# godhj93/bayesian-torch

Measured on AMD Instinct MI355X. Metric: MC-samples/sec (forward+KL), Bayesian-ResNet18 CIFAR batch=128, higher is better.
Workload: dtype f32 (bf16x3 split operands, 6 product terms, f32 accumulate); 1 GPU; cfg3: Bayesian-ResNet18 via dnn_to_bnn (Conv2dReparameterization), CIFAR 3x32x32, batch=128; samples_per_launch=32, batch=128, rng=on-chip philox, parallelism=mc1, output_stage=bn+relu+residual (+ the stem max-pool) folded into the conv kernels, launch=hip graph replay

## Files before the change

### bayesian_torch_amd/_lib.py

```python
import ctypes as C
import os
import threading

import torch

_HERE = os.path.dirname(os.path.abspath(__file__))
LIB_PATH = os.environ.get("BT_LIB_PATH") or os.path.join(_HERE, "libbtorch_hip.so")
WORKSPACE_BYTES = 65536
KL_MAX_SEGMENTS = 64
PACK_MAX_SEGMENTS = 64
KL_RHO_IS_SIGMA = 1
KL_PRIOR_LAPLACE = 2
PRIOR_NORMAL, PRIOR_LAPLACE = 0, 1
DRAWS_EPS_PACKED = 1
LOWRANK_MAX_R = 4
DRAWS_SIGNS_PACKED = 2


def signs_packed_stride(n):
    return (int(n) + 15) // 16 * 16

_f32p = C.POINTER(C.c_float)
_vp = C.c_void_p

# ... 56 lines not shown
class bt_minmax_seg(C.Structure):
    _fields_ = [("x", _vp), ("n", C.c_int64), ("dst", _vp)]


MINMAX_MAX_SEGS = 4

_lib = None
_lock = threading.Lock()

_FWD_TAIL = [_vp, C.c_int64, C.POINTER(bt_params), C.POINTER(bt_draws), C.POINTER(bt_epilogue), _vp, _vp, _vp, C.c_size_t, _vp]
_PROTOS = {
    "bt_version": (C.c_int, []),
    "bt_last_error_string": (C.c_char_p, []),
    "bt_last_kernel_name": (C.c_char_p, []),
    "bt_last_launch_info": (C.c_int, [C.POINTER(C.c_int64), C.c_int32]),
    "bt_fused_scratch_bytes": (C.c_size_t, [C.POINTER(bt_conv2d_geom), C.c_int32]),
    "bt_set_contraction": (C.c_int, [C.c_int]),
    "bt_get_contraction": (C.c_int, []),
    "bt_conv2d_bwd_workspace": (C.c_size_t, [C.POINTER(bt_conv2d_geom), C.c_int32]),
    "bt_conv2d_bwd": (C.c_int, [C.POINTER(bt_conv2d_geom), C.c_int32, C.c_int32, _vp, C.c_int64, _vp, C.POINTER(bt_params), C.POINTER(bt_draws),
                                _vp, _vp, _vp, _vp, C.c_size_t, _vp]),
    "bt_maxpool_3x3s2": (C.c_int, [_vp, _vp, C.c_int64, C.c_int32, C.c_int32, _vp]),
    "bt_conv2d_bwd_kl": (C.c_int, [C.POINTER(bt_conv2d_geom), C.c_int32, C.c_int32, _vp, C.c_int64, _vp, C.POINTER(bt_params), C.POINTER(bt_draws), _vp,
                                   _vp, _vp, _vp, _vp, C.c_size_t, _vp]),
    "bt_kl_normal_bwd": (C.c_int, [_vp, _vp, _vp, _vp, _vp, C.c_int64, C.c_uint32, _vp, _vp, _vp]),
    "bt_kl_normal_bwd_segs": (C.c_int, [C.c_int32, C.POINTER(_vp), C.POINTER(_vp), C.POINTER(_vp), C.POINTER(_vp), C.POINTER(C.c_int64), _vp, C.c_uint32,
                                        C.POINTER(_vp), C.POINTER(_vp), _vp]),
    "bt_reparam_linear_fwd": (C.c_int, [C.c_int32] * 4 + _FWD_TAIL),
    "bt_flipout_linear_fwd": (C.c_int, [C.c_int32] * 4 + _FWD_TAIL),
    "bt_reparam_conv2d_fwd": (C.c_int, [C.POINTER(bt_conv2d_geom), C.c_int32] + _FWD_TAIL),
# ... 72 lines not shown
                    fn = getattr(handle, name)
                    fn.restype, fn.argtypes = res, args
                _lib = handle
    return _lib


LAUNCH_INFO_FIELDS = ("workgroups", "m_tiles", "n_tiles", "S", "t_NI", "t_R", "t_Wt", "pixel_major", "row_tiles", "kl_slices", "groups", "n_bt", "n_rt", "n_ct", "fused_kl")


def last_launch_info():
    v = (C.c_int64 * 16)()
    check(lib().bt_last_launch_info(v, 16))
    return dict(zip(LAUNCH_INFO_FIELDS, (int(x) for x in v)))


ERR_UNSUPPORTED = -2


def check(rc):
    if rc != 0:
        raise RuntimeError(f"libbtorch_hip error {rc}: {lib().bt_last_error_string().decode()}")


def ptr(t):
    return None if t is None else t.data_ptr()


def dev_f32(t, what):
    if t is None:
        return None
# ... 96 lines not shown
```

### bayesian_torch_amd/csrc/bt_fused_api.hip

```cpp
#include <math.h>
#include <string.h>

#include "bt_fused_fwd.h"

namespace bt {
typedef int Launcher(bool linear, const FwdArgs& a, FwdArgs& ran, hipStream_t stream);
Launcher launch_reparam, launch_reparam_inj, launch_reparam_updil, launch_reparam_dwin, launch_flipout, launch_flipout_inj, launch_flipout_updil, launch_flipout_dwin;
static Launcher* const kLaunchers[2][4] = {{launch_reparam, launch_reparam_inj, launch_reparam_updil, launch_reparam_dwin},
                                           {launch_flipout, launch_flipout_inj, launch_flipout_updil, launch_flipout_dwin}};

EnvKnob g_force_generic{"BT_FORCE_GENERIC", [](const char* e) { return e ? 1 : 0; }};
static unsigned long long* g_dbg = nullptr;
static thread_local long long g_launch_info[16] = {};
static inline bool al16(const void* p) { return (((uintptr_t)p) & 15u) == 0; }
static void record_plan(const FwdArgs& r, int fused_kl) {
  const long long v[16] = {r.total_blocks, r.m_tiles, r.n_tiles, r.S, r.t_NI, r.t_R, r.t_Wt, r.pixel_major, r.row_taps, r.kl_slices, r.G, r.n_bt, r.n_rt, r.n_ct, fused_kl, 0};
  for (int i = 0; i < 16; ++i) g_launch_info[i] = v[i];
}

struct Call {
  bool flip, linear;
  const bt_conv2d_geom& g;
  int S;
  const float* x;
  int64_t x_sample_stride;
  const bt_params* p;
  const bt_draws* d;
  const bt_epilogue* ep;
  float *out, *kl_out;
  void* ws;
  size_t ws_bytes;
  const char* who;
  const bt_updil* u;
// ... 343 lines not shown
```

### bayesian_torch_amd/csrc/bt_fused_common.h

```cpp
#pragma once
#include "bt_api_internal.h"

namespace bt {

struct FwdArgs {
  const float *x, *mu_w, *rho_w, *mu_b, *rho_b, *pmu_w, *psig_w, *pmu_b, *psig_b;
  const float *mu_pk, *sig_pk;
  const float *eps_w, *eps_b, *sign_in, *sign_out;
  float* out;
  float* kl_out;
  double* slots;
  unsigned* counter;
  long long x_sample_stride, x_elems, out_elems, w_elems;
  int B, Ci, H, W, Co, KH, KW, SH, SW, PH, PW, DH, DW, G;
  int Ho, Wo, HoWo, M, K, Cig, Cog, S, T, HW;
  int n_tiles, m_tiles, total_blocks;
  int t_NI, t_R, t_Wt, n_bt, n_rt, n_ct;
  int patch_ok;
  int x_cvec;
  int x_rows;
  int pixel_major, mt_per_pixel;
  int w_vec, x_vec;
  int do_kl, kl_slices;
  uint32_t seed_lo, seed_hi, call, layer_id, sample0;
  const uint32_t* call_base;
  const float *ep_scale, *ep_shift, *ep_res;
  long long ep_res_stride;
  int ep_relu;
  int ep_pool, ep_Hp, ep_Wp;
  int out_vec4;
  int bn32;
  unsigned long long* dbg;
  uint32_t inv_m_tiles, inv_S, inv_n_tiles, inv_n_bt, inv_n_ct, inv_rw, inv_wt, inv_kw;
  int x_flat;
  int row_taps;
  float* sk_scratch;
  unsigned* sk_tickets;
  long long sk_scratch_bytes;
  int sk_nsl, sk_ks, sk_cpt;
// ... 21 lines not shown
  constexpr size_t end_dw = offsetof(FwdArgs, inv_do) + sizeof(uint32_t);
  constexpr size_t end_lr = offsetof(FwdArgs, lr_R) + sizeof(int);
  constexpr size_t end_obs = offsetof(FwdArgs, obs_nonfinite) + sizeof(unsigned*);
  static_assert(offsetof(FwdArgs, call_base) == hole + 4 && offsetof(FwdArgs, dwin) == end && offsetof(FwdArgs, lowrank) == end_dw &&
                    offsetof(FwdArgs, obs_dst) == end_lr && sizeof(FwdArgs) == end_obs,
                "FwdArgs padding moved: name the holes here");
  h = fnv1a(h, &a, hole);
  h = fnv1a(h, &a.call_base, end - offsetof(FwdArgs, call_base));
  if (a.dwin) h = fnv1a(h, &a.dwin, end_dw - end);
  if (a.lowrank) h = fnv1a(h, &a.lowrank, end_lr - end_dw);
  return a.obs_nonfinite ? fnv1a(h, &a.obs_dst, end_obs - end_lr) : h;
}

int launch_split(FwdArgs a, FwdArgs& ran, hipStream_t stream);
int launch_split_flip(FwdArgs a, FwdArgs& ran, hipStream_t stream);
int contraction_mode();
long long skinny_scratch_bytes(const bt_conv2d_geom& g, int S);

__device__ __forceinline__ RngKey weight_key(const FwdArgs& a) {
  RngKey key_w;
  key_w.seed_lo = a.seed_lo;
  key_w.seed_hi = a.seed_hi;
  key_w.call = a.call + (a.call_base ? __builtin_nontemporal_load(a.call_base) : 0u);
  key_w.layer_tensor = layer_tensor_word(a.layer_id, 0);
  return key_w;
}

__device__ __forceinline__ void sign_keys(const FwdArgs& a, const RngKey& key_w, uint32_t sample, uint32_t* skey_in, uint32_t* skey_out) {
  RngKey ks = key_w;
  ks.layer_tensor = layer_tensor_word(a.layer_id, 2);
// ... 103 lines not shown
  bt_ = wave_sum(bt_);
  if (lane == 0) {
    float kl = (float)(t / (double)a.w_elems);
    if (a.mu_b) kl += (float)(bt_ / (double)a.Co);
    a.kl_out[0] = kl;
    __hip_atomic_store(a.counter, 0u, __ATOMIC_RELAXED, __HIP_MEMORY_SCOPE_AGENT);
  }
}
__device__ __forceinline__ double kl_slot_sum(const FwdArgs& a, int nslots, int lane) {
  double t = 0.0;
  for (int q = lane; q < nslots; q += 64) t += __hip_atomic_load(&a.slots[q], __ATOMIC_RELAXED, __HIP_MEMORY_SCOPE_AGENT);
  for (int q = lane; q < nslots; q += 64) __hip_atomic_store(&a.slots[q], 0.0, __ATOMIC_RELAXED, __HIP_MEMORY_SCOPE_AGENT);
  return t;
}

struct ColDecode {
  int b0, r0, w0, RW, Mt, t_Wt;
  uint32_t inv_rw, inv_wt;
  int B, Ho, Wo;
  __device__ __forceinline__ bool decode(int ml, int& b, int& ho, int& wo) const {
    const int img = RW == 1 ? ml : (int)__umulhi((uint32_t)ml, inv_rw);
    const int rem = ml - img * RW;
    const int r = t_Wt == 1 ? rem : (int)__umulhi((uint32_t)rem, inv_wt);
    b = b0 + img, ho = r0 + r, wo = w0 + (rem - r * t_Wt);
    return ml < Mt && b < B && ho < Ho && wo < Wo;
  }
};

}
```

### bayesian_torch_amd/csrc/bt_fused_split.h

```cpp
#pragma once
#include "bt_fused_common.h"
#include "bt_fused_fwd.h"

namespace bt {

typedef short bf16x8 __attribute__((ext_vector_type(8)));

constexpr int kSplitSteps = 5;

template <int BM, bool FLIP = false>
constexpr int split_xpo() {
  return FLIP ? 302 : 1025;
}
template <int BN, int NP, bool FLIP = false>
constexpr int split_w_bytes() { return (FLIP ? 2 : 1) * kSplitSteps * 2 * NP * BN * 16; }
template <int BM, int NP, bool FLIP = false>
constexpr int split_x_bytes() { return split_xpo<BM, FLIP>() * (NP + (FLIP ? 1 : 0)) * 16; }
constexpr int kSplitMiscBytes = kMaxTaps * 16 + 96 + 32 + 64;
template <int BN, int BM, int NP, bool FLIP = false>
constexpr int split_stage_cap() {
  constexpr int ops = 2 * (split_w_bytes<BN, NP, FLIP>() + split_x_bytes<BM, NP, FLIP>()), pass32 = (4 * BN + 32 * (BM + 4)) * 4;
  return (NP == 1 && pass32 > ops) ? pass32 : ops;
}
template <int BN, int BM, int NP, bool FLIP = false>
// ... 30 lines not shown
  return inv ? (int)__umulhi((uint32_t)n, inv) : (d == 1 ? n : n / d);
}
__device__ __forceinline__ uint32_t inv32(int d) { return 0xFFFFFFFFu / (uint32_t)d + 1u; }
__device__ __forceinline__ int div_small(int n, int d) { return d == 1 ? n : d == 2 ? n >> 1 : n / d; }

#ifndef BT_ONE_PIXEL_STEPS
#define BT_ONE_PIXEL_STEPS 4
#endif
constexpr int kOnePixelSteps = BT_ONE_PIXEL_STEPS;

__device__ __forceinline__ uint32_t guarded_off(bool in, uint32_t off) {
  const uint32_t m = 0u - (uint32_t)in;
  return (off & m) | (0x80000000u & ~m);
}

__device__ __forceinline__ bool one_pixel_tile(const FwdArgs& a, int* tap) {
  if (a.HoWo != 1 || a.HW != 1 || a.t_R != 1 || a.t_Wt != 1 || a.m_tiles != a.n_bt || a.updil) return false;
  const int kh = a.DH == 1 ? a.PH : a.PH / a.DH, kw = a.DW == 1 ? a.PW : a.PW / a.DW;
  *tap = kh * a.KW + kw;
  return kh * a.DH == a.PH && kh < a.KH && kw * a.DW == a.PW && kw < a.KW && (a.Cig >> 3) > 0;
}

template <int BN, int NP, int NPW, bool INJ>
__device__ __forceinline__ void split_one_pixel_tile(const FwdArgs& a, const int tap) {
  constexpr int BM = 128, KS = kOnePixelSteps, kProducers = 64 * NPW, TN = BN / 32;
  constexpr int W_STEP = 2 * NP * BN * 16, W_HALF = NP * BN * 16, W_PIECE = BN * 16, W_RING = KS * W_STEP;
  constexpr int XD = 4;
  static_assert(KS % XD == 0, "whole groups per stage");
  static_assert(2 * W_RING + 3 * BN * 4 <= split_stage_cap<BN, BM, NP>(), "two weight images + the channel constants fit the operand buffers");
  extern __shared__ __attribute__((aligned(16))) char smem_c[];
  float* const bias0 = reinterpret_cast<float*>(smem_c + 2 * W_RING);
// ... 302 lines not shown
  const int mt = __builtin_amdgcn_readfirstlane(L - Lq * a.m_tiles);
  L = Lq, Lq = udiv_inv(L, a.S, a.inv_S);
  const int s = __builtin_amdgcn_readfirstlane(L - Lq * a.S);
  L = Lq, Lq = udiv_inv(L, a.n_tiles, a.inv_n_tiles);
  const int nt = __builtin_amdgcn_readfirstlane(L - Lq * a.n_tiles);
  const int g = __builtin_amdgcn_readfirstlane(Lq);
  const int n0 = nt * BN;
  const bool pix = a.pixel_major != 0;
  const int t_NI = a.t_NI, t_R = a.t_R, t_Wt = a.t_Wt, RW = t_R * t_Wt, Mt = t_NI * RW;
  const int trest = udiv_inv(mt, a.n_bt, a.inv_n_bt);
  const int bt = __builtin_amdgcn_readfirstlane(mt - trest * a.n_bt);
  const int rt = __builtin_amdgcn_readfirstlane(udiv_inv(trest, a.n_ct, a.inv_n_ct)), ct = __builtin_amdgcn_readfirstlane(trest - rt * a.n_ct);
  const int b0 = bt * t_NI, r0 = rt * t_R, w0 = ct * t_Wt;
  const uint32_t inv_rw = RW > 1 ? (a.inv_rw ? a.inv_rw : inv32(RW)) : 0u;
  const uint32_t inv_wt = t_Wt > 1 ? (a.inv_wt ? a.inv_wt : inv32(t_Wt)) : 0u;
  const ColDecode cols = {b0, r0, w0, RW, Mt, t_Wt, inv_rw, inv_wt, a.B, a.Ho, a.Wo};
  const uint32_t sample = a.sample0 + (uint32_t)s;
  const int T = a.T, Cig = a.Cig;

  const RngKey key_w = weight_key(a);
  uint32_t skey_in = 0, skey_out = 0;
  if constexpr (FLIP) sign_keys(a, key_w, sample, &skey_in, &skey_out);

  int nA, dymin, dymax, dxmin, dxmax;
  {
    bool act = false;
    int4 e = make_int4(0, 0, 0, 0);
    if (lane < T) {
      const int kh = udiv_inv(lane, a.KW, a.inv_kw), kw = lane - kh * a.KW;
      e = make_int4(0, kh * a.DH, kw * a.DW, lane);
      if (pix) {
// ... 144 lines not shown
      for (int u = 0; u < U; ++u) {
        if (relu) v[u].x = v[u].x < 0.f ? 0.f : v[u].x, v[u].y = v[u].y < 0.f ? 0.f : v[u].y, v[u].z = v[u].z < 0.f ? 0.f : v[u].z, v[u].w = v[u].w < 0.f ? 0.f : v[u].w;
        if (okq[u]) *reinterpret_cast<float4*>(out_s + oidx[u]) = v[u];
      }
    }
  };

  const bool stage_cols = !a.out_vec4 && !pix && !a.row_taps && a.Ho * a.Wo > 4;
  auto readout_cols = [&](int pass, int t0) {
    constexpr int SROW = BM + 4, NT_ = kThreadsAll;
    static_assert(NT_ % BM == 0, "a thread keeps its column");
    constexpr int RSTEP = NT_ / BM, NITc = (SROWS + RSTEP - 1) / RSTEP;
    const float* const stage = smem + 4 * BN;
    const int c = t0 % BM, row0 = t0 / BM;
    int bq, hq, wq;
    const bool mok = cols.decode(c, bq, hq, wq);
    const int HoWo_ = a.Ho * a.Wo;
    const int co0 = pass * SROWS + row0;
    const uint32_t obase = mok ? (uint32_t)(((bq * a.Co + g * a.Cog + n0 + co0) * a.Ho + hq) * a.Wo + wq) : 0u;
    const int rows_ok = a.Cog - n0 - pass * SROWS < SROWS ? a.Cog - n0 - pass * SROWS : SROWS;
    const float* const sp = stage + row0 * SROW + c;
#pragma unroll 8
    for (int k = 0; k < NITc; ++k) {
      const int row = row0 + k * RSTEP;
      const bool ok = mok && row < rows_ok;
      const uint32_t oi = ok ? obase + (uint32_t)(k * RSTEP * HoWo_) : 0u;
      const int rr = row < SROWS ? k * RSTEP : 0;
      float v = sp[rr * SROW];
      if constexpr (FLIP) {
        const float d = sp[(SROWS + rr) * SROW];
        const int co_l = ok ? co0 + k * RSTEP : 0;
// ... 424 lines not shown
    auto kl_ticket = [&]() {
      int last = 0;
      if (lane == 0) last = (__hip_atomic_fetch_add(a.counter, 1u, __ATOMIC_RELAXED, __HIP_MEMORY_SCOPE_AGENT) == (unsigned)a.kl_slices - 1u) ? 1 : 0;
      if (__builtin_amdgcn_readfirstlane(last))
        kl_close(a, kl_slot_sum(a, 4 * a.kl_slices, lane), lane);
    };
    int xaddr[TM][kSplitSteps];
    {
      int pimg[TM], pyb[TM], pxb[TM];
      bool live[TM];
#pragma unroll
      for (int j = 0; j < TM; ++j) {
        int b, ho, wo;
        live[j] = cols.decode(wm * WTM + j * 32 + li, b, ho, wo);
        pimg[j] = (b - b0) * PIMG, pyb[j] = (ho - r0) * ps_h, pxb[j] = (wo - w0) * ps_w;
      }
#pragma unroll
      for (int q = 0; q < kSplitSteps; ++q) {
        int ol, ai;
        if (nA <= 1) ol = 2 * q + lh, ai = 0;
        else ol = (q >= SPO) + (q >= 2 * SPO) + (q >= 3 * SPO) + (q >= 4 * SPO), ai = 2 * (q - ol * SPO) + lh;
        const bool ent = nA > 0 && ol < NO && ai < nA;
        const int4 e = taptab[ent ? ai : 0];
        const int ty = (dymax == dymin) ? 0 : e.y - dymin, tx = (dxmax == dxmin) ? 0 : e.z - dxmin;
#pragma unroll
        for (int j = 0; j < TM; ++j) {
          const int yy = pyb[j] + ty, xx = pxb[j] + tx;
          const bool ok = ent && live[j] && yy >= kmin_h && yy <= kmax_h && xx >= kmin_w && xx <= kmax_w;
          xaddr[j][q] = ok ? (ol * PCH + pimg[j] + (yy - kmin_h) * NXR + (xx - kmin_w)) * PB : ZOFF;
        }
      }
    }
    int wlq[kSplitSteps];
#pragma unroll
    for (int q = 0; q < kSplitSteps; ++q) wlq[q] = lh * W_HALF + (li ^ ((2 * q + lh) & 7)) * 16 + wn * TN * 32 * 16;

    f32x16 acc[NOP][TN][TM];
#pragma unroll
    for (int o = 0; o < NOP; ++o)
#pragma unroll
      for (int i = 0; i < TN; ++i)
#pragma unroll
        for (int j = 0; j < TM; ++j)
#pragma unroll
          for (int r = 0; r < 16; ++r) acc[o][i][j][r] = 0.f;
    if (prio_mode == 2) __builtin_amdgcn_s_setprio(3);

// ... 33 lines not shown
#pragma unroll
        for (int q = 0; q < kSplitSteps; ++q) {
          if (q < nstep) {
#pragma unroll
            for (int j = 0; j < TM; ++j) {
              const int u = q * TM + j;
              if (j + 1 < TM) {
                read_x(u + 1);
              } else if (q + 1 < kSplitSteps) {
                if (q + 1 < nstep) {
                  read_x(u + 1);
                  read_w(q + 1);
                }
              }
              __builtin_amdgcn_sched_barrier(0);
#pragma unroll
              for (int o = 0; o < NOP; ++o) {
                if (o == 1) {
#pragma unroll
                  for (int p = 0; p < NP; ++p) xf[u & 1][p] ^= xf[u & 1][NXP - 1];
                }
#pragma unroll
                for (int i = 0; i < TN; ++i) {
                  acc[o][i][j] = __builtin_amdgcn_mfma_f32_32x32x16_bf16(xf[u & 1][0], wf[q & 1][o][i][0], acc[o][i][j], 0, 0, 0);
                  if constexpr (NP >= 2) {
                    acc[o][i][j] = __builtin_amdgcn_mfma_f32_32x32x16_bf16(xf[u & 1][0], wf[q & 1][o][i][1], acc[o][i][j], 0, 0, 0);
                    acc[o][i][j] = __builtin_amdgcn_mfma_f32_32x32x16_bf16(xf[u & 1][1], wf[q & 1][o][i][0], acc[o][i][j], 0, 0, 0);
                  }
                  if constexpr (NP == 3) {
                    acc[o][i][j] = __builtin_amdgcn_mfma_f32_32x32x16_bf16(xf[u & 1][0], wf[q & 1][o][i][2], acc[o][i][j], 0, 0, 0);
                    acc[o][i][j] = __builtin_amdgcn_mfma_f32_32x32x16_bf16(xf[u & 1][1], wf[q & 1][o][i][1], acc[o][i][j], 0, 0, 0);
                    acc[o][i][j] = __builtin_amdgcn_mfma_f32_32x32x16_bf16(xf[u & 1][2], wf[q & 1][o][i][0], acc[o][i][j], 0, 0, 0);
                  }
                }
              }
              __builtin_amdgcn_sched_barrier(0);
            }
          }
        }
      }
      if (cstamp && st < 60) dbg_[2 + 2 * st + 1] = __builtin_amdgcn_s_memtime();
      if (kl_block) kls.group(a);
      __syncthreads();
    }
    if (kl_block) kl_finish();
    if (cstamp) dbg_[1] = __builtin_amdgcn_s_memtime();
    __syncthreads();
    if (kl_block && wave == 0) kl_ticket();
    if (cstamp) dbg_[120] = __builtin_amdgcn_s_memtime();

// ... 59 lines not shown
        float v = __fadd_rn(acc[0][i][j][r], bsv[i]);
        if constexpr (SGN) v = __fadd_rn(v, __fmul_rn(__fadd_rn(acc[NOP - 1][i][j][r], b1v[i]), so_f((uint32_t)so_s[oi], 0)));
        else if constexpr (FLIP) v = __fadd_rn(v, __fmul_rn(__fadd_rn(acc[NOP - 1][i][j][r], b1v[i]), hash_sign(skey_out, oi)));
        return __fadd_rn(__fmul_rn(v, scv[i]), shv[i]);
      };
      if (a.row_taps && t_Wt == 2 && (a.Wo & 1) == 0 && (out_mis & 7u) == 0) {
#pragma unroll
        for (int j = 0; j < TM; ++j) {
          uint32_t base[8];
          bool live[8];
          float2 rr[8][TN];
#pragma unroll
          for (int r2 = 0; r2 < 8; ++r2) {
            const int r = 2 * r2, row = (r & 3) + 8 * (r >> 2) + 4 * lh;
            int bb, hh, ww;
            live[r2] = cols.decode(wm * WTM + j * 32 + row, bb, hh, ww);
            base[r2] = live[r2] ? (uint32_t)((bb * a.Co + g * a.Cog + n0) * HoWo + hh * a.Wo + ww) : 0u;
#pragma unroll
            for (int i = 0; i < TN; ++i) {
              rr[r2][i] = make_float2(0.f, 0.f);
              if (res_s && live[r2] && cok[i]) rr[r2][i] = *reinterpret_cast<const float2*>(res_s + base[r2] + (uint32_t)(((wn * TN + i) * 32 + li) * HoWo));
            }
          }
#pragma unroll
          for (int r2 = 0; r2 < 8; ++r2) {
            const int r = 2 * r2;
#pragma unroll
            for (int i = 0; i < TN; ++i) {
              if (live[r2] && cok[i]) {
                const uint32_t oi = base[r2] + (uint32_t)(((wn * TN + i) * 32 + li) * HoWo);
                float v0 = outv(i, j, r, oi), v1 = outv(i, j, r + 1, oi + 1u);
// ... 2 lines not shown
                *reinterpret_cast<float2*>(out_s + oi) = make_float2(v0, v1);
              }
            }
          }
        }
      } else if (!pix && !a.row_taps && HoWo == 4 && t_R == a.Ho && t_Wt == a.Wo && (out_mis & 15u) == 0) {
#pragma unroll
        for (int j = 0; j < TM; ++j) {
          uint32_t base[4];
          bool live[4];
          float4 rr[4][TN];
#pragma unroll
          for (int q = 0; q < 4; ++q) {
            const int row = 8 * q + 4 * lh;
            int bb, hh, ww;
            live[q] = cols.decode(wm * WTM + j * 32 + row, bb, hh, ww);
            base[q] = live[q] ? (uint32_t)((bb * a.Co + g * a.Cog + n0) * HoWo) : 0u;
#pragma unroll
            for (int i = 0; i < TN; ++i) {
              rr[q][i] = make_float4(0.f, 0.f, 0.f, 0.f);
              if (res_s && live[q] && cok[i]) rr[q][i] = *reinterpret_cast<const float4*>(res_s + base[q] + (uint32_t)(((wn * TN + i) * 32 + li) * HoWo));
            }
          }
#pragma unroll
          for (int q = 0; q < 4; ++q) {
#pragma unroll
            for (int i = 0; i < TN; ++i) {
              if (live[q] && cok[i]) {
                const uint32_t oi = base[q] + (uint32_t)(((wn * TN + i) * 32 + li) * HoWo);
                float v[4];
#pragma unroll
// ... 4 lines not shown
                *reinterpret_cast<float4*>(out_s + oi) = make_float4(v[0], v[1], v[2], v[3]);
              }
            }
          }
        }
      } else
#pragma unroll
      for (int j = 0; j < TM; ++j) {
        uint32_t base[16];
        bool live[16];
        float rr[16][TN];
#pragma unroll
        for (int r = 0; r < 16; ++r) {
          const int row = (r & 3) + 8 * (r >> 2) + 4 * lh;
          int bb, hh, ww;
          live[r] = cols.decode(wm * WTM + j * 32 + row, bb, hh, ww);
          base[r] = live[r] ? (uint32_t)((bb * a.Co + g * a.Cog + n0) * HoWo + hh * a.Wo + ww) : 0u;
#pragma unroll
          for (int i = 0; i < TN; ++i) {
            rr[r][i] = 0.f;
            if (res_s && live[r] && cok[i]) rr[r][i] = res_s[base[r] + (uint32_t)(((wn * TN + i) * 32 + li) * HoWo)];
          }
        }
#pragma unroll
        for (int r = 0; r < 16; ++r) {
#pragma unroll
          for (int i = 0; i < TN; ++i) {
            if (live[r] && cok[i]) {
              const uint32_t oi = base[r] + (uint32_t)(((wn * TN + i) * 32 + li) * HoWo);
              float v = outv(i, j, r, oi);
              if (res_s) v = __fadd_rn(v, rr[r][i]);
// ... 17 lines not shown
```

### bayesian_torch_amd/csrc/bt_fused_split.hip

```cpp
#include <stdlib.h>
#include <string.h>

#include "bt_fused_split_host.h"
#include "bt_fused_split_launch.h"

namespace bt {

static EnvKnob g_contraction{"BT_CONTRACTION", [](const char* e) { return !e ? 0 : (!strcmp(e, "f32") ? 1 : !strcmp(e, "bf16x2") ? 2 : !strcmp(e, "bf16") ? 3 : 0); }};
int contraction_mode() { return g_contraction.get(); }
EnvKnob g_bn32{"BT_BN32", [](const char* e) { return e ? (atoi(e) ? 1 : 0) : -1; }};
static EnvKnob g_direct_off{nullptr, [](const char*) { return 0; }};
static EnvKnob g_skinny_off{"BT_NO_SKINNY", [](const char* e) { return (e && *e && *e != '0') ? 1 : 0; }};

static int quad_spw(const FwdArgs& a, long long tiles, int mode) {
  if (a.eps_w) return 0;
  if (mode == 3) return 0;
  if (!a.ep_pool || a.x_sample_stride != 0 || a.S < 2 || a.Ho != 16 || a.Wo != 16 || a.t_NI != 2 || a.ep_Hp != 8 || a.ep_Wp != 8) return 0;
  int nd[2] = {};
  tap_window(a.KH, a.DH, a.SH, a.PH, a.H, a.Ho, false, &nd[0], &nd[1]);
  int nw, dxs;
  tap_window(a.KW, a.DW, a.SW, a.PW, a.W, a.Wo, false, &nw, &dxs);
  const long long PHt = 15ll * (nd[1] ? a.SH : 1) + nd[1] + 1, PWt = 15ll * (dxs ? a.SW : 1) + dxs + 1;
  if (2 * PHt * PWt * 24 + kWalkBytes > kQuadXBytes) return 0;
  static int n_cu[64] = {};
  int dev = 0;
// ... 134 lines not shown
    const int rc = launch_split_one(t, ran, stream);
    if (rc <= 0) return rc;
  }
  const int rc = launch_split_one(a, ran, stream);
  if (rc != 1 || !a.pixel_major) return rc;
  a.pixel_major = 0;
  a.out_vec4 = 0;
  return launch_split_one(a, ran, stream);
}

}

extern "C" void bt_debug_disable_direct(int off) { bt::g_direct_off.set(off ? 1 : 0); }
extern "C" void bt_debug_force_bn32(int v) { bt::g_bn32.set(v < 0 ? -1 : (v ? 1 : 0)); }
extern "C" void bt_debug_disable_skinny(int off) { bt::g_skinny_off.set(off ? 1 : 0); }

extern "C" int bt_set_contraction(int mode) {
  if (mode < 0 || mode > 3) return bt::set_error(BT_ERR_BAD_ARG, "bt_set_contraction: mode must be 0 (auto), 1 (f32), 2 (bf16x2) or 3 (bf16)");
  bt::g_contraction.set(mode);
  return BT_OK;
}
extern "C" int bt_get_contraction(void) { return bt::contraction_mode(); }
```

### bayesian_torch_amd/csrc/bt_fused_split_host.h

```cpp
#pragma once
#include <stdlib.h>

#include "bt_fused_split.h"

namespace bt {

extern EnvKnob g_bn32;

static inline uint32_t inv_u32(long long d, long long nmax) {
  if (d <= 1 || nmax < 0 || (unsigned long long)nmax * (unsigned long long)d >= (1ull << 32)) return 0u;
  return (uint32_t)(((1ull << 32) + (unsigned long long)d - 1ull) / (unsigned long long)d);
}
static inline void split_fill_inverses(FwdArgs& a) {
  static const bool off = getenv("BT_NO_HOST_INV") != nullptr;
  if (off) {
    a.inv_m_tiles = a.inv_S = a.inv_n_tiles = a.inv_n_bt = a.inv_n_ct = a.inv_rw = a.inv_wt = a.inv_kw = a.inv_n_sg = a.inv_uh = a.inv_uw = a.inv_kd = a.inv_do = 0u;
    return;
  }
  const long long tb = a.total_blocks;
  a.inv_m_tiles = inv_u32(a.m_tiles, tb);
  a.inv_S = inv_u32(a.S, tb);
  a.inv_n_tiles = inv_u32(a.n_tiles, tb);
  a.inv_n_bt = inv_u32(a.n_bt, a.m_tiles);
  a.inv_n_ct = inv_u32(a.n_ct, a.m_tiles);
// ... 123 lines not shown
  int xm = 0;
  if (a.HW == 1) xm = 1;
  else if (bm != 128 && !a.pixel_major && a.HW > 1 && (a.W & 3) == 0 && a.t_Wt == a.Wo && split_row_mode(a)) xm = split_row_mode(a);
  else if constexpr (!FLIP) {
    if (bm != 128 && !a.pixel_major && a.HW > 1 && split_plane_flat(a)) xm = 3, a.x_flat = 1;
    else if (bm == 128 && !a.pixel_major && a.H == 2 && a.W == 2 && split_plane_flat(a)) xm = 2;
    else if (bm != 512 && a.row_taps && a.H == 2 && a.W == 2 && a.KW == 3 && a.PW == 1 && a.SW == 1 && a.DW == 1) xm = 2;
    else if (a.pixel_major && a.H == 2 && a.W == 2 && a.KH == 3 && a.KW == 3 && a.PH == 1 && a.PW == 1 && a.SH == 1 && a.SW == 1 && a.DH == 1 && a.DW == 1) xm = 2;
  }
  if constexpr (FLIP) {
    if (bm == 256 ? !(xm == 3 && a.SH == 1 && a.SW == 1) : xm != 1) xm = 0;
  }
  return xm;
}

template <bool FLIP>
static int split_plan(FwdArgs& a, int mode, int* bm_out, int* xm_out) {
  if (a.T > 9) return 1;
  const int Mdom = a.pixel_major ? a.B : a.M;
  if (Mdom < 112) return 1;
  a.n_tiles = (a.Cog + 63) / 64;
  FwdArgs cand[3] = {a, a, a};
  int live[3] = {0, 0, 0};
  if constexpr (!FLIP) {
    if (Mdom >= 512) live[0] = split_geometry<512>(cand[0]);
  }
  if (Mdom >= 256 && !(FLIP && a.pixel_major)) live[1] = split_geometry<256, FLIP>(cand[1]);
  live[2] = split_geometry<128, FLIP>(cand[2]);
  double cost[3];
  for (int i = 0; i < 3; ++i) cost[i] = split_tile_cost(cand[i], live[i], kSplitWidths[i], split_synth<FLIP>(kSplitWidths[i]), split_fixed<FLIP>());
  int pick = -1;
  if constexpr (!FLIP) {
    static const int force_bm = [] { const char* e = getenv("BT_FORCE_BM"); return e ? atoi(e) : 0; }();
    for (int i = 0; i < 3; ++i)
      if (force_bm == kSplitWidths[i] && cost[i] < 1e30) pick = i;
  }
  for (int i = 0; i < 3 && pick < 0; ++i) {
    bool best = cost[i] < 1e30;
    for (int j = i + 1; j < 3; ++j) best = best && cost[i] <= cost[j];
    if (best) pick = i;
  }
  if (pick < 0) return 1;
  const int bm = kSplitWidths[pick];
  const long long per = (long long)a.G * a.n_tiles * a.S;
  a = cand[pick];
  if constexpr (!FLIP) {
    a.bn32 = 0;
    if (bm == 128 && mode != 2 && a.Cog > 32) {
      const int forced = g_bn32.get();
      a.bn32 = forced >= 0 ? forced : (2 * per * a.m_tiles <= 256 ? 1 : 0);
    }
    if (a.bn32) a.n_tiles = (a.Cog + 31) / 32;
  }
  if (!set_grid(a, (long long)a.G * a.n_tiles * a.S * a.m_tiles)) return 1;
  *bm_out = bm, *xm_out = split_x_mode<FLIP>(a, bm);
  split_fill_inverses(a);
  return BT_OK;
}

}
```

### include/bt_hip.h

```cpp
#ifndef BT_HIP_H
#define BT_HIP_H

#include <stddef.h>
#include <stdint.h>

#ifdef __cplusplus
extern "C" {
#endif

#define BT_VERSION 302
#define BT_WORKSPACE_BYTES 65536

#define BT_OK 0
#define BT_ERR_BAD_ARG (-1)
#define BT_ERR_UNSUPPORTED (-2)
#define BT_ERR_WORKSPACE (-3)
#define BT_ERR_HIP_BASE (-1000)

typedef void *bt_stream_t;

typedef struct bt_rng {
  uint64_t seed;
  const uint32_t *call_base_dev;
  uint32_t call;
// ... 34 lines not shown
  const float *residual;
  int64_t residual_sample_stride;
  int32_t relu;
  int32_t pool;
} bt_epilogue;

#define BT_POOL_NONE 0
#define BT_POOL_MAX_3x3_S2_P1 1

int bt_version(void);
const char *bt_last_error_string(void);
const char *bt_last_kernel_name(void);
size_t bt_fused_scratch_bytes(const bt_conv2d_geom *g, int32_t S);

int bt_last_launch_info(int64_t *out, int32_t n);

int bt_reparam_linear_fwd(int32_t B, int32_t In, int32_t Out, int32_t S,
                          const float *x, int64_t x_sample_stride,
                          const bt_params *p, const bt_draws *d, const bt_epilogue *ep ,
                          float *out , float *kl_out ,
                          void *workspace, size_t workspace_bytes, bt_stream_t stream);

int bt_reparam_conv2d_fwd(const bt_conv2d_geom *g, int32_t S,
                          const float *x, int64_t x_sample_stride,
                          const bt_params *p, const bt_draws *d, const bt_epilogue *ep ,
                          float *out , float *kl_out,
                          void *workspace, size_t workspace_bytes, bt_stream_t stream);

typedef struct bt_updil {
  int32_t uh, uw;
// ... 216 lines not shown
```

Measured before the change: 18440 MC-samples/s.

## Skip MFMA units whose operand columns are entirely zero padding in split conv

Adds a per-wave dead-unit mask, built with ballots over the im2col addresses, and skips the MFMA work for units whose whole 32-column slice reads only padding (ZOFF). It also adds an optional row-grouped column decode that packs several images per 32-column block when Wo divides 32, which makes more units fully padded and so skippable. A host-side model picks the grouping only if it predicts more skipped units. The costs are extra ballot and decode arithmetic, a branch inside the inner MFMA loop that may upset scheduling, and a new debug query API.

```diff
diff --git a/bayesian_torch_amd/_lib.py b/bayesian_torch_amd/_lib.py
--- a/bayesian_torch_amd/_lib.py
+++ b/bayesian_torch_amd/_lib.py
@@ -94,6 +94,7 @@
     "bt_last_error_string": (C.c_char_p, []),
     "bt_last_kernel_name": (C.c_char_p, []),
     "bt_last_launch_info": (C.c_int, [C.POINTER(C.c_int64), C.c_int32]),
+    "bt_last_launch_skip": (C.c_int, [C.POINTER(C.c_int64), C.c_int32]),
     "bt_fused_scratch_bytes": (C.c_size_t, [C.POINTER(bt_conv2d_geom), C.c_int32]),
     "bt_set_contraction": (C.c_int, [C.c_int]),
     "bt_get_contraction": (C.c_int, []),
@@ -196,6 +197,15 @@
     return dict(zip(LAUNCH_INFO_FIELDS, (int(x) for x in v)))
 
 
+LAUNCH_SKIP_FIELDS = ("row_grouped", "ib", "units", "skipped_fastest", "skipped_slowest", "skipped_w0", "skipped_w1", "skipped_w2", "skipped_w3")
+
+
+def last_launch_skip():
+    v = (C.c_int64 * 9)()
+    check(lib().bt_last_launch_skip(v, 9))
+    return dict(zip(LAUNCH_SKIP_FIELDS, (int(x) for x in v)))
+
+
 ERR_UNSUPPORTED = -2
 
 
diff --git a/bayesian_torch_amd/csrc/bt_fused_api.hip b/bayesian_torch_amd/csrc/bt_fused_api.hip
--- a/bayesian_torch_amd/csrc/bt_fused_api.hip
+++ b/bayesian_torch_amd/csrc/bt_fused_api.hip
@@ -13,10 +13,13 @@
 static unsigned long long* g_dbg = nullptr;
 static thread_local long long g_launch_info[16] = {};
 static inline bool al16(const void* p) { return (((uintptr_t)p) & 15u) == 0; }
+static thread_local FwdArgs g_last_plan = {};
 static void record_plan(const FwdArgs& r, int fused_kl) {
   const long long v[16] = {r.total_blocks, r.m_tiles, r.n_tiles, r.S, r.t_NI, r.t_R, r.t_Wt, r.pixel_major, r.row_taps, r.kl_slices, r.G, r.n_bt, r.n_rt, r.n_ct, fused_kl, 0};
   for (int i = 0; i < 16; ++i) g_launch_info[i] = v[i];
-}
+  g_last_plan = r;
+}
+const FwdArgs& last_plan() { return g_last_plan; }
 
 struct Call {
   bool flip, linear;
diff --git a/bayesian_torch_amd/csrc/bt_fused_common.h b/bayesian_torch_amd/csrc/bt_fused_common.h
--- a/bayesian_torch_amd/csrc/bt_fused_common.h
+++ b/bayesian_torch_amd/csrc/bt_fused_common.h
@@ -23,6 +23,7 @@
   int w_vec, x_vec;
   int do_kl, kl_slices;
   uint32_t seed_lo, seed_hi, call, layer_id, sample0;
+  int pad_skip;
   const uint32_t* call_base;
   const float *ep_scale, *ep_shift, *ep_res;
   long long ep_res_stride;
@@ -74,6 +75,7 @@
 
 int launch_split(FwdArgs a, FwdArgs& ran, hipStream_t stream);
 int launch_split_flip(FwdArgs a, FwdArgs& ran, hipStream_t stream);
+const FwdArgs& last_plan();
 int contraction_mode();
 long long skinny_scratch_bytes(const bt_conv2d_geom& g, int S);
 
@@ -207,6 +209,7 @@
   return t;
 }
 
+constexpr int kPadSkip = 0x100;
 struct ColDecode {
   int b0, r0, w0, RW, Mt, t_Wt;
   uint32_t inv_rw, inv_wt;
@@ -219,5 +222,20 @@
     return ml < Mt && b < B && ho < Ho && wo < Wo;
   }
 };
-
-}
+struct ColDecodeRG : ColDecode {
+  int ib;
+  __device__ __forceinline__ ColDecodeRG(const ColDecode& c, int ib_) : ColDecode(c), ib(ib_) {}
+  __device__ __forceinline__ bool decode(int ml, int& b, int& ho, int& wo) const {
+    const int wsh = __builtin_ctz((unsigned)t_Wt | 32u), k = ml >> 5, low = ml & 31;
+    const int blk = (int)__umulhi((uint32_t)(k << wsh), inv_rw);
+    int img = RW == 1 ? ml : (int)__umulhi((uint32_t)ml, inv_rw);
+    const int rem = ml - img * RW;
+    int r = t_Wt == 1 ? rem : (int)__umulhi((uint32_t)rem, inv_wt);
+    int w = rem - r * t_Wt;
+    img = ib ? blk * ib + (low >> wsh) : img, r = ib ? k - blk * (RW >> wsh) : r, w = ib ? (low & (t_Wt - 1)) : w;
+    b = b0 + img, ho = r0 + r, wo = w0 + w;
+    return ml < Mt && b < B && ho < Ho && wo < Wo;
+  }
+};
+
+}
diff --git a/bayesian_torch_amd/csrc/bt_fused_split.h b/bayesian_torch_amd/csrc/bt_fused_split.h
--- a/bayesian_torch_amd/csrc/bt_fused_split.h
+++ b/bayesian_torch_amd/csrc/bt_fused_split.h
@@ -1,4 +1,6 @@
 #pragma once
+#include <type_traits>
+
 #include "bt_fused_common.h"
 #include "bt_fused_fwd.h"
 
@@ -68,7 +70,7 @@
   return (off & m) | (0x80000000u & ~m);
 }
 
-__device__ __forceinline__ bool one_pixel_tile(const FwdArgs& a, int* tap) {
+__host__ __device__ __forceinline__ bool one_pixel_tile(const FwdArgs& a, int* tap) {
   if (a.HoWo != 1 || a.HW != 1 || a.t_R != 1 || a.t_Wt != 1 || a.m_tiles != a.n_bt || a.updil) return false;
   const int kh = a.DH == 1 ? a.PH : a.PH / a.DH, kw = a.DW == 1 ? a.PW : a.PW / a.DW;
   *tap = kh * a.KW + kw;
@@ -401,7 +403,11 @@
   const int b0 = bt * t_NI, r0 = rt * t_R, w0 = ct * t_Wt;
   const uint32_t inv_rw = RW > 1 ? (a.inv_rw ? a.inv_rw : inv32(RW)) : 0u;
   const uint32_t inv_wt = t_Wt > 1 ? (a.inv_wt ? a.inv_wt : inv32(t_Wt)) : 0u;
-  const ColDecode cols = {b0, r0, w0, RW, Mt, t_Wt, inv_rw, inv_wt, a.B, a.Ho, a.Wo};
+  const ColDecode cols_im = {b0, r0, w0, RW, Mt, t_Wt, inv_rw, inv_wt, a.B, a.Ho, a.Wo};
+  const std::conditional_t<FLIP, ColDecode, ColDecodeRG> cols = [&] {
+    if constexpr (FLIP) return cols_im;
+    else return ColDecodeRG(cols_im, a.pad_skip & 0xFF);
+  }();
   const uint32_t sample = a.sample0 + (uint32_t)s;
   const int T = a.T, Cig = a.Cig;
 
@@ -576,7 +582,7 @@
     const float* const stage = smem + 4 * BN;
     const int c = t0 % BM, row0 = t0 / BM;
     int bq, hq, wq;
-    const bool mok = cols.decode(c, bq, hq, wq);
+    const bool mok = cols_im.decode(c, bq, hq, wq);
     const int HoWo_ = a.Ho * a.Wo;
     const int co0 = pass * SROWS + row0;
     const uint32_t obase = mok ? (uint32_t)(((bq * a.Co + g * a.Cog + n0 + co0) * a.Ho + hq) * a.Wo + wq) : 0u;
@@ -1031,6 +1037,7 @@
         int b, ho, wo;
         live[j] = cols.decode(wm * WTM + j * 32 + li, b, ho, wo);
         pimg[j] = (b - b0) * PIMG, pyb[j] = (ho - r0) * ps_h, pxb[j] = (wo - w0) * ps_w;
+
       }
 #pragma unroll
       for (int q = 0; q < kSplitSteps; ++q) {
@@ -1048,6 +1055,17 @@
         }
       }
     }
+    static_assert(kSplitSteps * TM <= 32, "the dead-unit mask is one word");
+    constexpr bool kSkipDead = !FLIP;
+    uint32_t dead = 0;
+    if (kSkipDead && (a.pad_skip & kPadSkip)) {
+#pragma unroll
+      for (int q = 0; q < kSplitSteps; ++q)
+#pragma unroll
+        for (int j = 0; j < TM; ++j) dead |= (__ballot(xaddr[j][q] != ZOFF) == 0ull ? 1u : 0u) << (q * TM + j);
+    }
+    dead = __builtin_amdgcn_readfirstlane(dead);
+    if constexpr (kSkipDead) asm volatile("" : "+s"(dead));
     int wlq[kSplitSteps];
 #pragma unroll
     for (int q = 0; q < kSplitSteps; ++q) wlq[q] = lh * W_HALF + (li ^ ((2 * q + lh) & 7)) * 16 + wn * TN * 32 * 16;
@@ -1111,6 +1129,7 @@
                 }
               }
               __builtin_amdgcn_sched_barrier(0);
+              if (!kSkipDead || !(dead & (1u << u))) {
 #pragma unroll
               for (int o = 0; o < NOP; ++o) {
                 if (o == 1) {
@@ -1131,6 +1150,7 @@
                   }
                 }
               }
+              }
               __builtin_amdgcn_sched_barrier(0);
             }
           }
@@ -1220,7 +1240,7 @@
           for (int r2 = 0; r2 < 8; ++r2) {
             const int r = 2 * r2, row = (r & 3) + 8 * (r >> 2) + 4 * lh;
             int bb, hh, ww;
-            live[r2] = cols.decode(wm * WTM + j * 32 + row, bb, hh, ww);
+            live[r2] = cols_im.decode(wm * WTM + j * 32 + row, bb, hh, ww);
             base[r2] = live[r2] ? (uint32_t)((bb * a.Co + g * a.Cog + n0) * HoWo + hh * a.Wo + ww) : 0u;
 #pragma unroll
             for (int i = 0; i < TN; ++i) {
@@ -1253,7 +1273,7 @@
           for (int q = 0; q < 4; ++q) {
             const int row = 8 * q + 4 * lh;
             int bb, hh, ww;
-            live[q] = cols.decode(wm * WTM + j * 32 + row, bb, hh, ww);
+            live[q] = cols_im.decode(wm * WTM + j * 32 + row, bb, hh, ww);
             base[q] = live[q] ? (uint32_t)((bb * a.Co + g * a.Cog + n0) * HoWo) : 0u;
 #pragma unroll
             for (int i = 0; i < TN; ++i) {
@@ -1288,7 +1308,7 @@
         for (int r = 0; r < 16; ++r) {
           const int row = (r & 3) + 8 * (r >> 2) + 4 * lh;
           int bb, hh, ww;
-          live[r] = cols.decode(wm * WTM + j * 32 + row, bb, hh, ww);
+          live[r] = cols_im.decode(wm * WTM + j * 32 + row, bb, hh, ww);
           base[r] = live[r] ? (uint32_t)((bb * a.Co + g * a.Cog + n0) * HoWo + hh * a.Wo + ww) : 0u;
 #pragma unroll
           for (int i = 0; i < TN; ++i) {
diff --git a/bayesian_torch_amd/csrc/bt_fused_split.hip b/bayesian_torch_amd/csrc/bt_fused_split.hip
--- a/bayesian_torch_amd/csrc/bt_fused_split.hip
+++ b/bayesian_torch_amd/csrc/bt_fused_split.hip
@@ -9,6 +9,8 @@
 static EnvKnob g_contraction{"BT_CONTRACTION", [](const char* e) { return !e ? 0 : (!strcmp(e, "f32") ? 1 : !strcmp(e, "bf16x2") ? 2 : !strcmp(e, "bf16") ? 3 : 0); }};
 int contraction_mode() { return g_contraction.get(); }
 EnvKnob g_bn32{"BT_BN32", [](const char* e) { return e ? (atoi(e) ? 1 : 0) : -1; }};
+EnvKnob g_pad_skip{"BT_PAD_SKIP", [](const char* e) { return e ? (atoi(e) ? 1 : 0) : 1; }};
+EnvKnob g_force_bm{"BT_FORCE_BM", [](const char* e) { return e ? atoi(e) : 0; }};
 static EnvKnob g_direct_off{nullptr, [](const char*) { return 0; }};
 static EnvKnob g_skinny_off{"BT_NO_SKINNY", [](const char* e) { return (e && *e && *e != '0') ? 1 : 0; }};
 
@@ -173,6 +175,28 @@
 extern "C" void bt_debug_disable_direct(int off) { bt::g_direct_off.set(off ? 1 : 0); }
 extern "C" void bt_debug_force_bn32(int v) { bt::g_bn32.set(v < 0 ? -1 : (v ? 1 : 0)); }
 extern "C" void bt_debug_disable_skinny(int off) { bt::g_skinny_off.set(off ? 1 : 0); }
+extern "C" void bt_debug_force_pad_skip(int on) { bt::g_pad_skip.set(on ? 1 : 0); }
+extern "C" void bt_debug_force_bm(int bm) { bt::g_force_bm.set(bm > 0 ? bm : 0); }
+
+extern "C" int bt_last_launch_skip(int64_t* out, int32_t n) {
+  if (!out || n <= 0) return bt::set_error(BT_ERR_BAD_ARG, "bt_last_launch_skip: bad argument");
+  int64_t v[9] = {};
+  const char* name = bt_last_kernel_name();
+  const bt::FwdArgs& r = bt::last_plan();
+  int bn = 0, bm = 0, tap;
+  if (name && sscanf(name, "fused_split_kernel<%d,%d,", &bn, &bm) == 2 && (bm == 128 || bm == 256 || bm == 512)) {
+    const bool flip = strstr(name, ",flip") != nullptr;
+    if (!(strstr(name, "xm=1") && !flip && bt::one_pixel_tile(r, &tap))) {
+      const int ib = r.pad_skip & 0xFF;
+      const bt::SkipModel m = bt::split_skip_model(r, bm, flip, ib, r.B);
+      const bool on = (r.pad_skip & bt::kPadSkip) != 0;
+      v[0] = ib ? 1 : 0, v[1] = ib, v[2] = m.units, v[3] = on ? m.most() : 0, v[4] = on ? m.fewest() : 0;
+      for (int w = 0; w < 4; ++w) v[5 + w] = on ? m.skipped[w] : 0;
+    }
+  }
+  for (int i = 0; i < n; ++i) out[i] = i < 9 ? v[i] : 0;
+  return BT_OK;
+}
 
 extern "C" int bt_set_contraction(int mode) {
   if (mode < 0 || mode > 3) return bt::set_error(BT_ERR_BAD_ARG, "bt_set_contraction: mode must be 0 (auto), 1 (f32), 2 (bf16x2) or 3 (bf16)");
diff --git a/bayesian_torch_amd/csrc/bt_fused_split_host.h b/bayesian_torch_amd/csrc/bt_fused_split_host.h
--- a/bayesian_torch_amd/csrc/bt_fused_split_host.h
+++ b/bayesian_torch_amd/csrc/bt_fused_split_host.h
@@ -6,6 +6,8 @@
 namespace bt {
 
 extern EnvKnob g_bn32;
+extern EnvKnob g_pad_skip;
+extern EnvKnob g_force_bm;
 
 static inline uint32_t inv_u32(long long d, long long nmax) {
   if (d <= 1 || nmax < 0 || (unsigned long long)nmax * (unsigned long long)d >= (1ull << 32)) return 0u;
@@ -161,6 +163,81 @@
   return xm;
 }
 
+struct SkipModel {
+  int units, skipped[4];
+  int fewest() const { int m = skipped[0]; for (int w = 1; w < 4; ++w) m = skipped[w] < m ? skipped[w] : m; return m; }
+  int most() const { int m = skipped[0]; for (int w = 1; w < 4; ++w) m = skipped[w] > m ? skipped[w] : m; return m; }
+};
+static SkipModel split_skip_model(const FwdArgs& a, int bm, bool flip, int ib, int b_lim) {
+  SkipModel m = {0, {0, 0, 0, 0}};
+  const int CWM = flip ? 2 : 4, WTM = bm / CWM, TM = WTM / 32;
+  const int t_R = a.t_R, t_Wt = a.t_Wt, RW = t_R * t_Wt, Mt = a.t_NI * RW;
+  int ey[kMaxTaps], ex[kMaxTaps], nA = 0, dymin = 1 << 20, dymax = -1, dxmin = 1 << 20, dxmax = -1;
+  for (int t = 0; t < a.T && t < kMaxTaps; ++t) {
+    const int y = (t / a.KW) * a.DH, x = (t % a.KW) * a.DW;
+    bool act;
+    if (a.pixel_major) {
+      act = (unsigned)(-a.PH + y) < (unsigned)a.H && (unsigned)(-a.PW + x) < (unsigned)a.W;
+    } else {
+      const int lo_h = a.PH - y, lo_w = a.PW - x;
+      const int hc = lo_h > 0 ? (lo_h + a.SH - 1) / a.SH : 0, wc = lo_w > 0 ? (lo_w + a.SW - 1) / a.SW : 0;
+      act = hc < a.Ho && hc * a.SH - lo_h < a.H && wc < a.Wo && wc * a.SW - lo_w < a.W;
+      if (a.row_taps) act = act && (unsigned)(-a.PH + y) < (unsigned)a.H;
+    }
+    if (!act) continue;
+    ey[nA] = y, ex[nA] = x, ++nA;
+    dymin = y < dymin ? y : dymin, dymax = y > dymax ? y : dymax, dxmin = x < dxmin ? x : dxmin, dxmax = x > dxmax ? x : dxmax;
+  }
+  if (!nA) return m;
+  const int ps_h = dymax == dymin ? 1 : a.SH, gs_h = dymax == dymin ? a.SH : 1, ps_w = dxmax == dxmin ? 1 : a.SW, gs_w = dxmax == dxmin ? a.SW : 1;
+  const int PHt = (t_R - 1) * ps_h + (dymax - dymin) + 1, PWt = (t_Wt - 1) * ps_w + (dxmax - dxmin) + 1;
+  const int x_lo = -a.PW + dxmin, y_lo = -a.PH + dymin;
+  const int kmin_h = y_lo < 0 ? (-y_lo + gs_h - 1) / gs_h : 0, kmin_w = x_lo < 0 ? (-x_lo + gs_w - 1) / gs_w : 0;
+  int kmax_h = a.H - 1 - y_lo >= 0 ? (a.H - 1 - y_lo) / gs_h : -1, kmax_w = a.W - 1 - x_lo >= 0 ? (a.W - 1 - x_lo) / gs_w : -1;
+  kmax_h = kmax_h < PHt - 1 ? kmax_h : PHt - 1, kmax_w = kmax_w < PWt - 1 ? kmax_w : PWt - 1;
+  const int NYR = kmax_h >= kmin_h ? kmax_h - kmin_h + 1 : 0, NXR = kmax_w >= kmin_w ? kmax_w - kmin_w + 1 : 0;
+  const int PCH = a.t_NI * NYR * NXR, XPO = flip ? split_xpo<256, true>() : split_xpo<512, false>(), G8 = a.Cig >> 3, SPO = (nA + 1) >> 1;
+  int NO = nA <= 1 ? 2 * kSplitSteps : (SPO == 1 ? 5 : SPO == 2 ? 2 : 1);
+  while (NO > 1 && NO * PCH > XPO - 1) --NO;
+  if (nA <= 1 && NO > 1) NO &= ~1;
+  if (NO > G8) NO = G8;
+  const int NSTEP = nA <= 1 ? (NO + 1) >> 1 : NO * SPO;
+  m.units = NSTEP * TM;
+  for (int w = 0; w < 4; ++w) {
+    const int wm = w & (CWM - 1);
+    for (int q = 0; q < NSTEP; ++q)
+      for (int j = 0; j < TM; ++j) {
+        bool any = false;
+        for (int lane = 0; lane < 64 && !any; ++lane) {
+          const int li = lane & 31, lh = lane >> 5;
+          const int ol = nA <= 1 ? 2 * q + lh : q / SPO, ai = nA <= 1 ? 0 : 2 * (q - ol * SPO) + lh;
+          if (ol >= NO || ai >= nA) continue;
+          const int ml = wm * WTM + j * 32 + li;
+          int b, ho, wo;
+          if (ib) {
+            const int k = ml >> 5, low = ml & 31, blk = k / t_R;
+            b = blk * ib + low / t_Wt, ho = k - blk * t_R, wo = low % t_Wt;
+          } else {
+            const int img = ml / RW, rem = ml - img * RW;
+            b = img, ho = rem / t_Wt, wo = rem - ho * t_Wt;
+          }
+          if (!(ml < Mt && b < b_lim && ho < a.Ho && wo < a.Wo)) continue;
+          const int yy = ho * ps_h + (dymax == dymin ? 0 : ey[ai] - dymin), xx = wo * ps_w + (dxmax == dxmin ? 0 : ex[ai] - dxmin);
+          any = yy >= kmin_h && yy <= kmax_h && xx >= kmin_w && xx <= kmax_w;
+        }
+        if (!any) ++m.skipped[w];
+      }
+  }
+  return m;
+}
+static int split_row_group(const FwdArgs& a, int bm, bool flip) {
+  if (a.pixel_major || a.row_taps || !a.out_vec4 || a.HoWo == 1) return 0;
+  if (a.t_R != a.Ho || a.t_Wt != a.Wo || (a.Wo & 3) || a.Wo > 32 || 32 % a.Wo) return 0;
+  const int ib = 32 / a.Wo;
+  if (a.t_NI % ib) return 0;
+  return split_skip_model(a, bm, flip, ib, a.t_NI).fewest() > split_skip_model(a, bm, flip, 0, a.t_NI).fewest() ? ib : 0;
+}
+
 template <bool FLIP>
 static int split_plan(FwdArgs& a, int mode, int* bm_out, int* xm_out) {
   if (a.T > 9) return 1;
@@ -177,8 +254,8 @@
   double cost[3];
   for (int i = 0; i < 3; ++i) cost[i] = split_tile_cost(cand[i], live[i], kSplitWidths[i], split_synth<FLIP>(kSplitWidths[i]), split_fixed<FLIP>());
   int pick = -1;
-  if constexpr (!FLIP) {
-    static const int force_bm = [] { const char* e = getenv("BT_FORCE_BM"); return e ? atoi(e) : 0; }();
+  {
+    const int force_bm = g_force_bm.get();
     for (int i = 0; i < 3; ++i)
       if (force_bm == kSplitWidths[i] && cost[i] < 1e30) pick = i;
   }
@@ -201,6 +278,7 @@
   }
   if (!set_grid(a, (long long)a.G * a.n_tiles * a.S * a.m_tiles)) return 1;
   *bm_out = bm, *xm_out = split_x_mode<FLIP>(a, bm);
+  a.pad_skip = (!FLIP && g_pad_skip.get()) ? (kPadSkip | split_row_group(a, bm, FLIP)) : 0;
   split_fill_inverses(a);
   return BT_OK;
 }
diff --git a/include/bt_hip.h b/include/bt_hip.h
--- a/include/bt_hip.h
+++ b/include/bt_hip.h
@@ -72,6 +72,7 @@
 size_t bt_fused_scratch_bytes(const bt_conv2d_geom *g, int32_t S);
 
 int bt_last_launch_info(int64_t *out, int32_t n);
+int bt_last_launch_skip(int64_t *out, int32_t n);
 
 int bt_reparam_linear_fwd(int32_t B, int32_t In, int32_t Out, int32_t S,
                           const float *x, int64_t x_sample_stride,
```

Measured after the change: 18600 MC-samples/s, median of 6. About the same (+0.9%).
